# BioinfoMachineLearning/bio-diffusion

Hardware: NVIDIA H100
Metric: molecules/sec (1000-step sample) (higher is better)
Workload: dtype bf16x2 (split hi+lo operands, f32 accumulate; <=1e-4 of the fp32 reference)

## Files before the change

bio-diffusion_b200/csrc/bdiff_edge_tc.cuh:

```cuda
#pragma once
#include "bdiff_kernels.h"
#include "bdiff_slab.cuh"

namespace bdiff {

constexpr int TMT = 128;
constexpr int TC_SLOT = 2 * 160 * 32;
constexpr int TC_NSLOT = 5;
constexpr int TM_S = 0, TM_U0 = 256, TM_U1 = 288, TM_MV = 320, TM_VD0 = 416;
constexpr int TM_EX = 416, TM_EX_STRIDE = 40;

struct StreamSeg { int steps, rows, group; };
struct Stream { StreamSeg seg[8]; int n; };
__host__ __device__ constexpr int seg_step_bytes(StreamSeg g) { return 2 * g.rows * 32; }
__host__ __device__ constexpr int seg_chunks(StreamSeg g) { return (g.steps + g.group - 1) / g.group; }
__host__ __device__ constexpr size_t stream_bytes(const Stream& s) {
  size_t b = 0;
  for (int i = 0; i < s.n; ++i) b += (size_t)s.seg[i].steps * 2 * seg_step_bytes(s.seg[i]);
  return b;
}
__host__ __device__ constexpr long long stream_plane_rows(const Stream& s) {
  long long r = 0;
  for (int i = 0; i < s.n; ++i) r += (long long)s.seg[i].steps * 2 * s.seg[i].rows;
  return r;
}
__host__ __device__ constexpr int stream_max_chunk(const Stream& s) {
  int m = 0;
  for (int i = 0; i < s.n; ++i) {
    const int c = s.seg[i].group * seg_step_bytes(s.seg[i]);
    m = c > m ? c : m;
  }
  return m;
}

__host__ __device__ constexpr int tc_k0_steps(int Ed, int Xd) {
  return (Ed + (64 + Xd) / 4 + 9 + 15) / 16;
}
__host__ __device__ constexpr Stream tc_edge_stream(int k0s) {
  constexpr StreamSeg Ga{16, 160, 1}, Gb{2, 128, 1};
  return {{{k0s, 128, 1}, Ga, Gb, Ga, Gb, Ga, Gb, {16, 16, 4}}, 8};
}
static_assert(stream_max_chunk(tc_edge_stream(8)) <= TC_SLOT, "an edge-pass chunk must fit a ring slot");

struct TcBars {
  uint64_t full[TC_NSLOT], empty[TC_NSLOT], wbar;
  uint64_t item_full[2], item_empty[2], tile_done;
  alignas(16) int item[2][4];
};

constexpr int TC_EPI = 256;

struct alignas(16) SmallW {
  float Wd0x[16 * 20];
  float Wf0x[16 * 3];
  float Wu0[20 * 32];
  float Wdk[3][32 * 8];
  float Wfk[3][32 * 3];
  float Wuk[3][8 * 32];
  float bg[4][32];
  float bk[3][256];
  float wa[256];
  float ba[4];
};

struct EdgeTail : TcBars {
  float2 wbuf[2][8][2][32];
  SmallW sw;
  float sAttn[2][TMT];
  int sRow[TMT], sCol[TMT], sB[TMT], sNa[TMT];
  uint32_t winfo[8];
};

template <int HP, bool FIRST, bool LAST>
__device__ __forceinline__ void gate_update(int half, int ucol, const float* __restrict__ vdp,
                                            const float* __restrict__ Wu, const float* __restrict__ bgp,
                                            const float* __restrict__ Wdn, const float* __restrict__ Wfn,
                                            float* __restrict__ part) {
  float2 p2[4][3];
  if (!LAST) {
#pragma unroll
    for (int i = 0; i < 33; ++i) part[i] = 0.f;
#pragma unroll
    for (int hp = 0; hp < 4; ++hp) { p2[hp][0] = make_float2(0.f, 0.f); p2[hp][1] = p2[hp][0]; p2[hp][2] = p2[hp][0]; }
  }
  for (int oc = half * 2; oc < half * 2 + 2; ++oc) {
    float u[8], mv[24];
    scratch_ld<8>(ucol + oc * 8, u);
    if (!FIRST) scratch_ld<24>(TM_MV + oc * 24, mv);
#pragma unroll
    for (int jp = 0; jp < 4; ++jp) {
      const int o = oc * 8 + 2 * jp;
      const float2 g = sigmoid_acc2(__fadd2_rn(make_float2(u[2 * jp], u[2 * jp + 1]),
                                               *reinterpret_cast<const float2*>(bgp + o)));
      float2 s0 = make_float2(0.f, 0.f), s1 = s0, s2 = s0;
#pragma unroll
      for (int h = 0; h < HP; ++h) {
        const float2 wu = *reinterpret_cast<const float2*>(Wu + h * 32 + o);
        s0 = __ffma2_rn(wu, make_float2(vdp[h * 3 + 0], vdp[h * 3 + 0]), s0);
        s1 = __ffma2_rn(wu, make_float2(vdp[h * 3 + 1], vdp[h * 3 + 1]), s1);
        s2 = __ffma2_rn(wu, make_float2(vdp[h * 3 + 2], vdp[h * 3 + 2]), s2);
      }
      const int ja = 2 * jp * 3, jb = (2 * jp + 1) * 3;
      float2 r0, r1, r2;
      if (FIRST) { r0 = __fmul2_rn(s0, g); r1 = __fmul2_rn(s1, g); r2 = __fmul2_rn(s2, g); }
      else {
        r0 = __ffma2_rn(s0, g, make_float2(mv[ja + 0], mv[jb + 0]));
        r1 = __ffma2_rn(s1, g, make_float2(mv[ja + 1], mv[jb + 1]));
        r2 = __ffma2_rn(s2, g, make_float2(mv[ja + 2], mv[jb + 2]));
      }
      mv[ja + 0] = r0.x; mv[jb + 0] = r0.y; mv[ja + 1] = r1.x; mv[jb + 1] = r1.y; mv[ja + 2] = r2.x; mv[jb + 2] = r2.y;
    }
    scratch_st<24>(TM_MV + oc * 24, mv);
    if (!LAST) {
#pragma unroll
      for (int j = 0; j < 8; ++j) {
        const int c = oc * 8 + j;
        const float4 wd0 = *reinterpret_cast<const float4*>(Wdn + c * 8), wd1 = *reinterpret_cast<const float4*>(Wdn + c * 8 + 4);
        const float2 wdp[4] = {make_float2(wd0.x, wd0.y), make_float2(wd0.z, wd0.w), make_float2(wd1.x, wd1.y),
                               make_float2(wd1.z, wd1.w)};
#pragma unroll
        for (int x = 0; x < 3; ++x) {
          const float2 mb = make_float2(mv[j * 3 + x], mv[j * 3 + x]);
#pragma unroll
          for (int hp = 0; hp < 4; ++hp) p2[hp][x] = __ffma2_rn(wdp[hp], mb, p2[hp][x]);
        }
#pragma unroll
        for (int ch = 0; ch < 3; ++ch) {
          const float wf = Wfn[c * 3 + ch];
          part[24 + ch * 3 + 0] = fmaf(wf, mv[j * 3 + 0], part[24 + ch * 3 + 0]);
          part[24 + ch * 3 + 1] = fmaf(wf, mv[j * 3 + 1], part[24 + ch * 3 + 1]);
          part[24 + ch * 3 + 2] = fmaf(wf, mv[j * 3 + 2], part[24 + ch * 3 + 2]);
        }
      }
    }
  }
  if (!LAST) {
#pragma unroll
    for (int hp = 0; hp < 4; ++hp)
#pragma unroll
      for (int x = 0; x < 3; ++x) { part[(2 * hp) * 3 + x] = p2[hp][x].x; part[(2 * hp + 1) * 3 + x] = p2[hp][x].y; }
  }
}

__device__ __forceinline__ void pair_exchange33(int half, const float* __restrict__ mine, float* __restrict__ theirs) {
  float pad[40];
#pragma unroll
  for (int i = 0; i < 33; ++i) pad[i] = mine[i];
#pragma unroll
  for (int i = 33; i < 40; ++i) pad[i] = 0.f;
  scratch_st<40>(TM_EX + half * TM_EX_STRIDE, pad);
  named_bar_sync(3, TC_EPI);
  float got[40];
  scratch_ld<40>(TM_EX + (half ^ 1) * TM_EX_STRIDE, got);
#pragma unroll
  for (int i = 0; i < 33; ++i) theirs[i] = got[i];
}

}
```

bio-diffusion_b200/csrc/bdiff_layers_tc.cu:

```cuda
#include <type_traits>

#include "bdiff_node_tc.cuh"

namespace bdiff {

__device__ __forceinline__ int ld_acquire_gpu(const int* p) {
  int v;
  asm volatile("ld.acquire.gpu.global.s32 %0, [%1];" : "=r"(v) : "l"(p) : "memory");
  return v;
}
__device__ __forceinline__ void st_release_gpu(int* p, int v) {
  asm volatile("st.release.gpu.global.s32 [%0], %1;" ::"l"(p), "r"(v) : "memory");
}

union LayersTail {
  TcBars bars;
  EdgeTail edge;
  NodeTail node;
};
constexpr size_t LAYERS_SMEM_BYTES = XE_BLOCKS * (size_t)X_BLOCK + TC_NSLOT * (size_t)TC_SLOT + sizeof(LayersTail) + 1024;
static_assert(LAYERS_SMEM_BYTES + 64 <= 232448, "shared memory budget of the layer megakernel (227 KiB per block)");

constexpr int LAYERS_THREADS = 384;
constexpr int LAYERS_REG_COMPUTE = 232, LAYERS_REG_SERVICE = 40;
static_assert(256 * LAYERS_REG_COMPUTE + 128 * LAYERS_REG_SERVICE <= 168 * LAYERS_THREADS, "setmaxnreg pool");
constexpr int RING_CONSUMERS = TC_EPI / 32;

struct AccToScratch {};
template <int NS, int NU, class Issue, class Epi = AccToScratch>
__device__ __forceinline__ void run_seg(TcBars& B, uint32_t raddr, uint32_t& ci, int nch, int scol, bool sfresh, int ucol,
                                        int ufresh, Issue&& issue, Epi&& epi = Epi{}) {
  constexpr int RS = NS ? NS / 2 : 1, RU = NU ? NU / 2 : 1;
  const int wg = threadIdx.x >> 7;
  const bool lead = (threadIdx.x & 31) == 0;
  for (int h = 0; h < 2; ++h) {
    float s[RS], u[RU];
    if (NS) {
      if (sfresh) {
#pragma unroll
        for (int i = 0; i < RS; ++i) s[i] = 0.f;
      } else {
        acc_load<NS>(s, scol + h * NS, wg);
      }
    }
    if (NU) {
      if ((ufresh >> h) & 1) {
#pragma unroll
        for (int i = 0; i < RU; ++i) u[i] = 0.f;
      } else {
        acc_load<NU>(u, ucol + h * NU, wg);
      }
    }
    for (int c = 0; c < nch; ++c) {
      const uint32_t slot = ci % TC_NSLOT;
      float ts[RS], tu[RU];
#pragma unroll
      for (int i = 0; i < RS; ++i) ts[i] = 0.f;
#pragma unroll
      for (int i = 0; i < RU; ++i) tu[i] = 0.f;
      mbar_wait(&B.full[slot], (ci / TC_NSLOT) & 1);
      wgmma_fence();
      issue(ts, tu, raddr + slot * TC_SLOT, c);
      wgmma_commit();
      wgmma_wait<0>();
      acc_fence<RS>(ts);
      acc_fence<RU>(tu);
      mbar_arrive_if(&B.empty[slot], lead);
      ++ci;
      if (NS) {
#pragma unroll
        for (int i = 0; i < RS; ++i) s[i] += ts[i];
      }
      if (NU) {
#pragma unroll
        for (int i = 0; i < RU; ++i) u[i] += tu[i];
      }
    }
    if constexpr (std::is_same_v<std::decay_t<Epi>, AccToScratch>) {
      if (NS) acc_store<NS>(s, scol + h * NS, wg);
      if (NU) acc_store<NU>(u, ucol + h * NU, wg);
    } else {
      epi(s, u, h, wg);
    }
  }
}

template <int ED, int XD>
__global__ void __launch_bounds__(LAYERS_THREADS, 1) k_layers_tc(Plan p, Dims d, EmbedW ew, LayerSched q, Work w) {
  constexpr int HID0 = (64 + XD) / 4;
  constexpr int H2 = HID0 / 2;
  constexpr int K0RAW = ED + HID0 + 9;
  constexpr int K0S = (K0RAW + 15) / 16;
  static_assert(HID0 % 2 == 0 && H2 * 3 <= 32 && HID0 + 9 <= 32 && ED % 16 == 0, "layout");

  extern __shared__ unsigned char smem_raw[];
  unsigned char* smem = smem_raw + ((1024u - (smem_u32(smem_raw) & 1023u)) & 1023u);
  unsigned char* X = smem;
  unsigned char* ring = smem + XE_BLOCKS * X_BLOCK;
  unsigned char* tail = ring + TC_NSLOT * TC_SLOT;
  TcBars& B = *reinterpret_cast<TcBars*>(tail);
  const int tid = threadIdx.x, warp = __shfl_sync(0xffffffffu, tid >> 5, 0), lane = tid & 31;
  const int hid0 = d.hid0;
  const int per_layer = q.TE + q.TN;
  const int total_items = q.nitems;
  int* const flags = q.sched + 2;

  if (tid == 0) {
    for (int i = 0; i < TC_NSLOT; ++i) { mbar_init(&B.full[i], 1); mbar_init(&B.empty[i], RING_CONSUMERS); }
    for (int i = 0; i < 2; ++i) { mbar_init(&B.item_full[i], 1); mbar_init(&B.item_empty[i], TC_EPI + 1); }
    mbar_init(&B.tile_done, TC_EPI);
    mbar_init(&B.wbar, 1);
    mbar_fence_init();
    acc_scratch = w.acc + (size_t)blockIdx.x * TM_COLS * 128;
  }
  __syncthreads();

  if (warp == 8) {
    asm volatile("setmaxnreg.dec.sync.aligned.u32 %0;\n" ::"n"(LAYERS_REG_SERVICE));
    if (lane == 0) {
      uint32_t ci = 0;
      for (uint32_t k = 0;; ++k) {
        const uint32_t slot = k & 1;
        mbar_wait_backoff(&B.item_empty[slot], ((k >> 1) & 1) ^ 1);
        int type = -1, layer = 0, tile = 0;
        for (;;) {
          const int qi = atomicAdd(q.sched, 1);
          if (qi >= 2 * total_items) break;
          const int it = __ldg(q.items + (qi >> 1));
          type = (it >> 30) & 1; layer = (it >> 24) & 63; tile = 2 * (it & 0xffffff) + (qi & 1);
          if (tile < (type == 0 ? q.TE : q.TN)) break;
          type = -1;
        }
        B.item[slot][0] = type; B.item[slot][1] = layer; B.item[slot][2] = tile;
        mbar_arrive(&B.item_full[slot]);
        if (type < 0) break;
        const size_t stride = type == 0 ? q.edge_blob_stride : q.node_blob_stride;
        const unsigned char* blob = (type == 0 ? q.edge_blob : q.node_blob) + (size_t)layer * stride;
        const Stream S = type == 0 ? tc_edge_stream(K0S) : tc_node_stream(layer == q.L - 1);
        size_t off = 0;
        for (int i = 0; i < S.n; ++i) {
          const StreamSeg g = S.seg[i];
          const uint32_t step = seg_step_bytes(g);
          for (int h = 0; h < 2; ++h)
            for (int c = 0; c < seg_chunks(g); ++c) {
              const int steps = min(g.group, g.steps - c * g.group);
              const uint32_t s = ci % TC_NSLOT;
              mbar_wait_backoff(&B.empty[s], ((ci / TC_NSLOT) & 1) ^ 1);
              mbar_expect_tx(&B.full[s], steps * step);
              bulk_g2s(ring + s * TC_SLOT, blob + h * (stride / 2) + off + (size_t)c * g.group * step, steps * step, &B.full[s]);
              ++ci;
            }
          off += (size_t)g.steps * step;
        }
      }
    }
  } else if (warp == 9) {
    asm volatile("setmaxnreg.dec.sync.aligned.u32 %0;\n" ::"n"(LAYERS_REG_SERVICE));
    if (lane == 0) {
      for (uint32_t k = 0;; ++k) {
        const uint32_t slot = k & 1;
        mbar_wait(&B.item_full[slot], (k >> 1) & 1);
        const int type = B.item[slot][0], layer = B.item[slot][1], tile = B.item[slot][2];
        if (type < 0) break;
        mbar_wait_backoff(&B.tile_done, k & 1);
        __threadfence();
        st_release_gpu(flags + (size_t)layer * per_layer + (type == 0 ? tile : q.TE + tile), 1);
        mbar_arrive(&B.item_empty[slot]);
      }
    }
  } else if (warp >= 10) {
    asm volatile("setmaxnreg.dec.sync.aligned.u32 %0;\n" ::"n"(LAYERS_REG_SERVICE));
  } else {
    asm volatile("setmaxnreg.inc.sync.aligned.u32 %0;\n" ::"n"(LAYERS_REG_COMPUTE));
    uint32_t pw = 0, ci = 0;
    int cur_type = -1, cur_layer = -1;
    const uint32_t xa = smem_u32(X) + (uint32_t)(tid >> 7) * 8192u;
    const uint32_t raddr = smem_u32(ring);
    int es = 0;
    long long* stamp = nullptr;
    auto PH = [&]() __attribute__((always_inline)) { if (stamp && tid == 0 && es < 32) stamp[es] = clock64(); ++es; };
    bool stamped[2] = {false, false};
    auto sz = [](int n) { return (uint32_t)((n * 4 + 15) & ~15); };
    for (uint32_t k = 0;; ++k) {
      const uint32_t slot = k & 1;
      mbar_wait(&B.item_full[slot], (k >> 1) & 1);
      const int type = __shfl_sync(0xffffffffu, B.item[slot][0], 0);
      const int layer = __shfl_sync(0xffffffffu, B.item[slot][1], 0);
      const int tile = __shfl_sync(0xffffffffu, B.item[slot][2], 0);
      if (type < 0) break;
      if (tid == 0 && w.dbg && k < 16) {
        w.dbg[(size_t)blockIdx.x * 64 + 4 * k] = (type << 30) | (layer << 24) | tile;
        w.dbg[(size_t)blockIdx.x * 64 + 4 * k + 1] = clock64();
      }
      if (type != cur_type || layer != cur_layer) {
        named_bar_sync(3, TC_EPI);
        if (tid == 0) {
          const LayerW lw = q.layers[layer];
          auto stage = [&](auto&& list) {
            uint32_t total = 0;
            list([&](float*, const float*, int n) { total += sz(n); });
            mbar_expect_tx(&B.wbar, total);
            list([&](float* dst, const float* src, int n) { bulk_g2s(dst, src, sz(n), &B.wbar); });
          };
          if (type == 0) {
            SmallW& s = reinterpret_cast<EdgeTail*>(tail)->sw;
            stage([&](auto&& cp) {
              cp(s.Wd0x, lw.Wd0x, XD * HID0); cp(s.Wf0x, lw.Wf0x, XD * 3); cp(s.Wu0, lw.Wu0, HID0 * 32);
              for (int kk = 0; kk < 3; ++kk) {
                cp(s.Wdk[kk], lw.Wdk[kk], 256); cp(s.Wuk[kk], lw.Wuk[kk], 256); cp(s.bk[kk], lw.bk[kk], 256);
                cp(s.Wfk[kk], lw.Wfk[kk], 96); cp(s.bg[kk + 1], lw.bgk[kk], 32);
              }
              cp(s.bg[0], lw.bg0, 32); cp(s.wa, lw.wa, 256); cp(s.ba, lw.ba, 1);
            });
          } else {
            const int last = layer == q.L - 1;
            const LayerW wn = q.layers[last ? layer : layer + 1];
            SmallWR4& s = reinterpret_cast<NodeTail*>(tail)->sw;
            stage([&](auto&& cp) {
              cp(s.Wdf, lw.Wdf, 64 * 16); cp(s.Wff, lw.Wff, 64 * 3); cp(s.Wuf, lw.Wuf, 16 * 32); cp(s.bgf, lw.bgf, 32);
              cp(s.b1, lw.b1, 256); cp(s.b2, lw.b2, 256);
              cp(s.Wdp, lw.Wdp, 32 * 8); cp(s.Wfp, lw.Wfp, 32 * 3); cp(s.Wup, lw.Wup, 8); cp(s.bp, lw.bp, 256);
              cp(s.wgp, lw.Wgp, 256); cp(s.bgp, lw.bgp, 1);
              if (!last) {
                cp(s.u.nx.b0, wn.b0, 256);
                cp(s.u.nx.Wd0i, wn.Wd0i, 32 * hid0); cp(s.u.nx.Wd0j, wn.Wd0j, 32 * hid0);
                cp(s.u.nx.Wf0i, wn.Wf0i, 96); cp(s.u.nx.Wf0j, wn.Wf0j, 96);
              } else {
                cp(s.u.pj.pWd, ew.pWd, 32 * 32); cp(s.u.pj.pWf, ew.pWf, 96); cp(s.u.pj.pbs, ew.pbs, d.Hin);
              }
            });
          }
        }
        mbar_wait(&B.wbar, pw);
        pw ^= 1;
        cur_type = type; cur_layer = layer;
      }
      if (tid == 0) {
        int lo = 0, hi = -1;
        const int* fbase = flags;
        if (type == 0) {
          if (layer > 0) {
            const int2 dep = q.edge_dep[tile];
            lo = dep.x; hi = dep.y;
            fbase = flags + (size_t)(layer - 1) * per_layer + q.TE;
          }
        } else {
          const int2 dep = q.node_dep[tile];
          lo = dep.x; hi = dep.y;
          fbase = flags + (size_t)layer * per_layer;
        }
        const long long t0 = clock64();
        for (int u = lo; u <= hi; ++u) {
          while (ld_acquire_gpu(fbase + u) == 0) {
            if (clock64() - t0 > (1ll << 32)) { atomicExch(q.err, 1); __threadfence_system(); __trap(); }
          }
        }
      }
      named_bar_sync(3, TC_EPI);
      __threadfence();
      if (tid == 0 && w.dbg && k < 16) w.dbg[(size_t)blockIdx.x * 64 + 4 * k + 2] = clock64();
      es = 0;
      stamp = nullptr;
      if (w.dbg && k >= 2 && !stamped[type]) { stamp = w.dbg + 256 * 64 + (size_t)blockIdx.x * 64 + type * 32; stamped[type] = true; }
      PH();
      const int last = type == 1 && layer == q.L - 1;
      int ph = 0;
      auto gemm = [&](int phase) __attribute__((always_inline)) {
        if (type == 0) {
          const int ph = phase;
#include "edge_tile_mma.inc"
        } else {
          const int ph = phase;
#include "node_r4_tile_mma.inc"
        }
      };
      auto run = [&]() __attribute__((always_inline)) { fence_proxy_async(); named_bar_sync(3, TC_EPI); PH(); gemm(ph++); };
      auto publish = [&]() __attribute__((always_inline)) { run(); named_bar_sync(3, TC_EPI); PH(); };
      auto release_u = [&]() __attribute__((always_inline)) { named_bar_sync(3, TC_EPI); gemm(-1); named_bar_sync(3, TC_EPI); };
      if (type == 0) {
        EdgeTail& T = *reinterpret_cast<EdgeTail*>(tail);
        const int half = tid >> 7, r = tid & 127;
        const SmallW& sw = T.sw;
#include "edge_tile_epilogue.inc"
      } else {
        NodeTail& T = *reinterpret_cast<NodeTail*>(tail);
        NodeScratch& SC = *reinterpret_cast<NodeScratch*>(X + R5_BLOCKS * R5_BLOCK);
        const int l = lane, s = warp, c0 = warp * 32;
        const SmallWR4& sw = T.sw;
#include "node_r4_tile_epilogue.inc"
      }
      PH();
      if (tid == 0 && w.dbg && k < 16) w.dbg[(size_t)blockIdx.x * 64 + 4 * k + 3] = clock64();
      mbar_arrive(&B.tile_done);
      mbar_arrive(&B.item_empty[slot]);
    }
  }
  __syncthreads();
}

bool tc_supported(int Ed, int Xd) { return (Ed == 64 && Xd == 16) || (Ed == 16 && Xd == 8); }

cudaError_t tc_layers_configure() {
  cudaError_t e = cudaFuncSetAttribute(k_layers_tc<64, 16>, cudaFuncAttributeMaxDynamicSharedMemorySize,
                                       (int)LAYERS_SMEM_BYTES);
  if (e != cudaSuccess) return e;
  return cudaFuncSetAttribute(k_layers_tc<16, 8>, cudaFuncAttributeMaxDynamicSharedMemorySize, (int)LAYERS_SMEM_BYTES);
}

void launch_layers_tc(cudaStream_t st, const Plan& p, const Dims& d, const EmbedW& ew, const LayerSched& q,
                      const Work& w, int num_sms) {
  const int grid = 2 * q.nitems < num_sms ? 2 * q.nitems : num_sms;
  if (d.Ed == 64) k_layers_tc<64, 16><<<grid, LAYERS_THREADS, LAYERS_SMEM_BYTES, st>>>(p, d, ew, q, w);
  else k_layers_tc<16, 8><<<grid, LAYERS_THREADS, LAYERS_SMEM_BYTES, st>>>(p, d, ew, q, w);
}

}
```

bio-diffusion_b200/csrc/bdiff_tc_pack.cu:

```cuda
#include "bdiff_node_tc.cuh"

namespace bdiff {

size_t tc_blob_bytes(int Ed, int Xd) { return stream_bytes(tc_edge_stream(tc_k0_steps(Ed, Xd))); }
size_t tc_node_blob_bytes() { return stream_bytes(tc_node_stream(false)); }

struct SlabPos {
  int seg, rows;
  int k0, n;
  int half, local;
  size_t base;
};
__device__ bool stream_find(const Stream& S, long long row, SlabPos& p) {
  size_t base = 0;
  for (int i = 0; i < S.n; ++i) {
    const StreamSeg g = S.seg[i];
    const long long seg_rows = (long long)g.steps * 2 * g.rows;
    if (row >= seg_rows) {
      row -= seg_rows;
      base += (size_t)g.steps * seg_step_bytes(g);
      continue;
    }
    const int step = (int)(row / (2 * g.rows)), n = (int)(row % (2 * g.rows));
    const int body = g.rows < 128 ? g.rows : 128, gate = g.rows - body;
    p.seg = i; p.rows = g.rows; p.k0 = step * 16; p.n = n;
    p.base = base + (size_t)step * seg_step_bytes(g);
    if (n < 2 * body) { p.half = n / body; p.local = n % body; }
    else { p.half = (n - 2 * body) / gate; p.local = body + (n - 2 * body) % gate; }
    return true;
  }
  return false;
}

__global__ void k_pack_edge_slabs(LayerW lw, Dims d, unsigned char* __restrict__ blob, size_t half_bytes) {
  const Stream S = tc_edge_stream(tc_k0_steps(d.Ed, d.Xd));
  const long long idx = (long long)blockIdx.x * blockDim.x + threadIdx.x;
  const int kk = (int)(idx & 15);
  SlabPos p;
  if (!stream_find(S, idx >> 4, p)) return;
  const int n = p.n, k = p.k0 + kk;
  float v;
  if (p.seg == 0) {
    v = k < d.K0 ? lw.W0e[(size_t)k * 256 + n] : 0.f;
  } else if (p.seg == 7) {
    v = lw.Wgk[2][(size_t)k * 32 + n];
  } else {
    const int gi = (p.seg - 1) >> 1;
    if (!(p.seg & 1)) {
      v = 256 + k < kKM ? lw.Wk[gi][(size_t)(256 + k) * 256 + n] : 0.f;
    } else if (n < 256) {
      v = lw.Wk[gi][(size_t)k * 256 + n];
    } else {
      const float* wprev = gi == 0 ? lw.Wg0 : lw.Wgk[gi - 1];
      const float* wthis = lw.Wgk[gi];
      const bool odd = ((gi + 1) & 1) != 0;
      const int c = (n - 256) & 31;
      v = (p.half == 0) == odd ? wprev[(size_t)k * 32 + c] : -wthis[(size_t)k * 32 + c];
    }
  }
  slab_store(blob + (size_t)p.half * half_bytes + p.base, p.rows, p.local, kk, v);
}

__global__ void k_pack_node_slabs(LayerW lw, LayerW wn, EmbedW ew, Dims d, int last, unsigned char* __restrict__ blob,
                                  size_t half_bytes) {
  const Stream S = tc_node_stream(last);
  const long long idx = (long long)blockIdx.x * blockDim.x + threadIdx.x;
  const int kk = (int)(idx & 15);
  SlabPos p;
  if (!stream_find(S, idx >> 4, p)) return;
  const int n = p.n, k = p.k0 + kk;
  float v;
  switch (p.seg) {
    case NG_1A: v = lw.W1[(size_t)k * 256 + n]; break;
    case NG_1B: v = n < 256 ? lw.W1[(size_t)(256 + k) * 256 + n] : -lw.Wgf[(size_t)k * 32 + (n - 256)]; break;
    case NG_1C: v = 512 + k < kKFF ? lw.W1[(size_t)(512 + k) * 256 + n] : 0.f; break;
    case NG_2: v = lw.W2[(size_t)k * 256 + n]; break;
    case NG_3A: v = n < 256 ? lw.Wp[(size_t)k * 256 + n] : lw.Wgf[(size_t)k * 32 + (n - 256)]; break;
    default:
      if (p.seg == (last ? NGL_3B : NG_3B)) v = 256 + k < kKM ? lw.Wp[(size_t)(256 + k) * 256 + n] : 0.f;
      else if (last) v = (k < 300 && n < d.Hin) ? ew.pWs[(size_t)k * d.Hin + n] : 0.f;
      else v = (p.seg == NG_4 ? wn.Wsi : wn.Wsj)[(size_t)k * 256 + n];
  }
  slab_store(blob + (size_t)p.half * half_bytes + p.base, p.rows, p.local, kk, v);
}

void launch_tc_pack(cudaStream_t st, const LayerW& lw, const Dims& d, unsigned char* blob) {
  const long long total = stream_plane_rows(tc_edge_stream(tc_k0_steps(d.Ed, d.Xd))) * 16;
  k_pack_edge_slabs<<<(unsigned)((total + 255) / 256), 256, 0, st>>>(lw, d, blob, tc_blob_bytes(d.Ed, d.Xd) / 2);
}

void launch_tc_pack_node(cudaStream_t st, const LayerW& lw, const LayerW& wn, const EmbedW& ew, const Dims& d, int last,
                         unsigned char* blob) {
  const long long total = stream_plane_rows(tc_node_stream(last)) * 16;
  k_pack_node_slabs<<<(unsigned)((total + 255) / 256), 256, 0, st>>>(lw, wn, ew, d, last, blob, tc_node_blob_bytes() / 2);
}

}
```

bio-diffusion_b200/csrc/edge_tile_epilogue.inc:

```
      const long long g = (long long)tile * TMT + r;
      constexpr int PV = HID0 * 3 + 9, PF4 = (PV + 3) / 4, PLD = PF4 * 4 + 1;
      constexpr int XF4 = XD * 3 / 4, XLD = XD * 3 + 1;
      constexpr int C0 = 128;
      static_assert(K0S <= 8 && 64 * (PLD + XLD) * 4 <= 2 * X_BLOCK, "staging areas");
      auto sFp = [&](int rr) { return reinterpret_cast<float*>(X + (rr >> 6) * XE_LO * X_BLOCK) + (rr & 63) * PLD; };
      auto sFx = [&](int rr) { return reinterpret_cast<float*>(X + (rr >> 6) * XE_LO * X_BLOCK) + 64 * PLD + (rr & 63) * XLD; };
      const int4 rc = __ldg(p.edge_rc + g);
      float f[9];
      {
        constexpr int F4_ROW = ED / 4;
        const float4* eb = reinterpret_cast<const float4*>(w.e + (size_t)tile * TMT * ED);
        const float4* xb = reinterpret_cast<const float4*>(w.xi + (size_t)tile * TMT * XD * 3);
        float4 ev[TMT * F4_ROW / TC_EPI], xv[TMT * XF4 / TC_EPI];
#pragma unroll
        for (int i = 0; i < TMT * F4_ROW / TC_EPI; ++i) ev[i] = eb[i * TC_EPI + tid];
#pragma unroll
        for (int i = 0; i < TMT * XF4 / TC_EPI; ++i) xv[i] = xb[i * TC_EPI + tid];
#pragma unroll
        for (int qq = 0; qq < 9; ++qq) f[qq] = w.frames[(size_t)g * 9 + qq];
        if (half == 0) { T.sRow[r] = rc.x; T.sCol[r] = rc.y; T.sB[r] = rc.z; T.sNa[r] = rc.w; }
#pragma unroll
        for (int i = 0; i < TMT * F4_ROW / TC_EPI; ++i) {
          const int idx = i * TC_EPI + tid;
          const int rr = idx / F4_ROW, kk = (idx % F4_ROW) * 4;
          xe_store4(X, rr, C0 + kk, ev[i].x, ev[i].y, ev[i].z, ev[i].w);
        }
#pragma unroll
        for (int i = 0; i < TMT * XF4 / TC_EPI; ++i) {
          const int idx = i * TC_EPI + tid;
          float* dst = sFx(idx / XF4) + (idx % XF4) * 4;
          dst[0] = xv[i].x; dst[1] = xv[i].y; dst[2] = xv[i].z; dst[3] = xv[i].w;
        }
      }
      const int row = rc.x;
      const float* pi = w.PI + (size_t)(row < 0 ? 0 : row) * kPStride;
      named_bar_sync(3, TC_EPI);
      {
        float4 pv[(TMT * PF4 + TC_EPI - 1) / TC_EPI];
#pragma unroll
        for (int i = 0; i < (TMT * PF4 + TC_EPI - 1) / TC_EPI; ++i) {
          const int idx = i * TC_EPI + tid;
          pv[i] = make_float4(0.f, 0.f, 0.f, 0.f);
          if (idx < TMT * PF4) {
            const int rr = idx / PF4, cj = T.sCol[rr];
            if (cj >= 0) pv[i] = *reinterpret_cast<const float4*>(w.PJ + (size_t)cj * kPStride + kH + (idx - rr * PF4) * 4);
          }
        }
        float vdh[32], vdf0[9];
#pragma unroll
        for (int i = 0; i < 32; ++i) vdh[i] = 0.f;
#pragma unroll
        for (int i = 0; i < 9; ++i) vdf0[i] = 0.f;
        if (row >= 0) {
#pragma unroll
          for (int i = 0; i < H2 * 3; ++i) vdh[i] = pi[kH + half * H2 * 3 + i];
          if (half == 0) {
#pragma unroll
            for (int i = 0; i < 9; ++i) vdf0[i] = pi[kH + HID0 * 3 + i];
          }
        }
        float xi[XD * 3];
#pragma unroll
        for (int c = 0; c < XD * 3; ++c) xi[c] = sFx(r)[c];
#pragma unroll
        for (int i = 0; i < (TMT * PF4 + TC_EPI - 1) / TC_EPI; ++i) {
          const int idx = i * TC_EPI + tid;
          if (idx < TMT * PF4) {
            const int rr = idx / PF4;
            float* dst = sFp(rr) + (idx - rr * PF4) * 4;
            dst[0] = pv[i].x; dst[1] = pv[i].y; dst[2] = pv[i].z; dst[3] = pv[i].w;
          }
        }
        named_bar_sync(3, TC_EPI);
        const float* pjv = sFp(r);
#pragma unroll
        for (int i = 0; i < H2 * 3; ++i) vdh[i] += pjv[half * H2 * 3 + i];
        if (half == 0) {
#pragma unroll
          for (int i = 0; i < 9; ++i) vdf0[i] += pjv[HID0 * 3 + i];
        }
#pragma unroll
        for (int c = 0; c < XD; ++c) {
#pragma unroll
          for (int h = 0; h < H2; ++h) {
            const float wd = sw.Wd0x[c * HID0 + half * H2 + h];
            vdh[h * 3 + 0] = fmaf(wd, xi[c * 3 + 0], vdh[h * 3 + 0]);
            vdh[h * 3 + 1] = fmaf(wd, xi[c * 3 + 1], vdh[h * 3 + 1]);
            vdh[h * 3 + 2] = fmaf(wd, xi[c * 3 + 2], vdh[h * 3 + 2]);
          }
        }
#pragma unroll
        for (int h = 0; h < H2; ++h)
          xe_store1(X, r, C0 + ED + half * H2 + h, safe_norm3(vdh[h * 3], vdh[h * 3 + 1], vdh[h * 3 + 2]));
        scratch_st<32>(TM_VD0 + half * 32, vdh);
        if (half == 0) {
#pragma unroll
          for (int c = 0; c < XD; ++c)
#pragma unroll
            for (int ch = 0; ch < 3; ++ch) {
              const float wf = sw.Wf0x[c * 3 + ch];
              vdf0[ch * 3 + 0] = fmaf(wf, xi[c * 3 + 0], vdf0[ch * 3 + 0]);
              vdf0[ch * 3 + 1] = fmaf(wf, xi[c * 3 + 1], vdf0[ch * 3 + 1]);
              vdf0[ch * 3 + 2] = fmaf(wf, xi[c * 3 + 2], vdf0[ch * 3 + 2]);
            }
#pragma unroll
          for (int ch = 0; ch < 3; ++ch)
#pragma unroll
            for (int ax = 0; ax < 3; ++ax)
              xe_store1(X, r, C0 + ED + HID0 + ch * 3 + ax,
                        f[ax * 3] * vdf0[ch * 3] + f[ax * 3 + 1] * vdf0[ch * 3 + 1] + f[ax * 3 + 2] * vdf0[ch * 3 + 2]);
#pragma unroll
          for (int i = HID0 + 9; i < K0S * 16 - ED; ++i) xe_store1(X, r, C0 + ED + i, 0.f);
        }
      }
      run();
      publish();

      float vd[24], vdf[9];
      for (int k = 1; k <= 3; ++k) {
        float part[33], other[33];
        if (k == 1) {
          float vd0[HID0 * 3];
          {
            float t0[64];
            float* t1 = t0 + 32;
            scratch_ld<64>(TM_VD0, t0);
#pragma unroll
            for (int i = 0; i < H2 * 3; ++i) { vd0[i] = t0[i]; vd0[H2 * 3 + i] = t1[i]; }
          }
          named_bar_sync(3, TC_EPI);
          gate_update<HID0, true, false>(half, TM_U0, vd0, sw.Wu0, sw.bg[0], sw.Wdk[0], sw.Wfk[0], part);
        } else {
          gate_update<8, false, false>(half, ((k - 1) & 1) ? TM_U1 : TM_U0, vd, sw.Wuk[k - 2], sw.bg[k - 1],
                                       sw.Wdk[k - 1], sw.Wfk[k - 1], part);
        }
        pair_exchange33(half, part, other);
#pragma unroll
        for (int i = 0; i < 24; ++i) vd[i] = half == 0 ? part[i] + other[i] : other[i] + part[i];
#pragma unroll
        for (int i = 0; i < 9; ++i) vdf[i] = half == 0 ? part[24 + i] + other[24 + i] : other[24 + i] + part[24 + i];
        {
          float a[16];
          if (half == 0) {
#pragma unroll
            for (int h = 0; h < 8; ++h) a[h] = safe_norm3(vd[h * 3], vd[h * 3 + 1], vd[h * 3 + 2]);
#pragma unroll
            for (int i = 0; i < 8; ++i) {
              const int ch = i / 3, ax = i - ch * 3;
              a[8 + i] = f[ax * 3] * vdf[ch * 3] + f[ax * 3 + 1] * vdf[ch * 3 + 1] + f[ax * 3 + 2] * vdf[ch * 3 + 2];
            }
          } else {
            a[0] = f[6] * vdf[6] + f[7] * vdf[7] + f[8] * vdf[8];
#pragma unroll
            for (int i = 1; i < 16; ++i) a[i] = 0.f;
          }
          xe_store8_extra(X, r, half * 16, a);
          xe_store8_extra(X, r, half * 16 + 8, a + 8);
        }
        run();
        publish();
      }
      const int wr0 = warp * 16;
      uint32_t m_start, m_end;
      {
        const int li = lane & 15, tr = wr0 + li;
        const int rw = T.sRow[tr];
        const int rp = tr > 0 ? T.sRow[tr - 1] : -2;
        const int rn = tr < TMT - 1 ? T.sRow[tr + 1] : -2;
        m_start = __ballot_sync(0xffffffffu, rw != rp) & 0xffffu;
        m_end = __ballot_sync(0xffffffffu, rw != rn && rw >= 0) & 0xffffu;
        if (lane == 0) T.winfo[warp] = m_start | (m_end << 16);
      }
      named_bar_sync(3, TC_EPI);
      const bool cutL = T.sB[0] != 0;
      const bool cutR = T.sRow[TMT - 1] >= 0 && T.sB[TMT - 1] != T.sNa[TMT - 1] - 1;
      const bool cont_in = !(m_start & 1u);
      float attw[16];
#pragma unroll
      for (int i = 0; i < 16; ++i) attw[i] = sigmoid_acc(T.sAttn[0][wr0 + i] + T.sAttn[1][wr0 + i] + sw.ba[0]);
      auto emit = [&](int trow, float2 val, int t, bool active) {
        if (!active) return;
        const bool l = cutL && (T.sRow[trow] == T.sRow[0]);
        const bool rr_ = cutR && (T.sRow[trow] == T.sRow[TMT - 1]);
        const size_t col = (size_t)t * 64 + 2 * lane;
        if (l && rr_) *reinterpret_cast<float2*>(w.mid + (size_t)tile * kMsg + col) = val;
        else if (l || rr_) atomicAdd(reinterpret_cast<float2*>(w.agg + (size_t)T.sRow[trow] * kMsg + col), val);
        else *reinterpret_cast<float2*>(w.agg + (size_t)T.sRow[trow] * kMsg + col) = val;
      };
      auto finish_crossing = [&](int t, bool active) {
        if (!(cont_in && (m_end & 0xffffu))) return;
        const float2 (*wb)[2][32] = T.wbuf[t & 1];
        int wa = warp - 1;
        while (wa > 0 && !(T.winfo[wa] & 0xffffu) && !(T.winfo[wa] >> 16)) --wa;
        float2 s = wb[wa][1][lane];
        for (int v2 = wa + 1; v2 < warp; ++v2) s = __fadd2_rn(s, wb[v2][1][lane]);
        s = __fadd2_rn(s, wb[warp][0][lane]);
        emit(wr0 + (__ffs(m_end & 0xffffu) - 1), s, t, active);
      };
      for (int t = 0; t < 4; ++t) {
        const unsigned char* xh_ = X + t * X_BLOCK + (lane & 3) * 4;
        const unsigned char* xl_ = X + (XE_LO + t) * X_BLOCK + (lane & 3) * 4;
        float2 acc = make_float2(0.f, 0.f);
        bool from_prev = cont_in;
        uint32_t hw[16], lw_[16];
#pragma unroll
        for (int i = 0; i < 16; ++i) {
          const int row_ = wr0 + i;
          const uint32_t off = (uint32_t)row_ * 128u + ((((uint32_t)lane >> 2) ^ ((uint32_t)row_ & 7u)) << 4);
          hw[i] = *reinterpret_cast<const uint32_t*>(xh_ + off);
          lw_[i] = *reinterpret_cast<const uint32_t*>(xl_ + off);
        }
#pragma unroll
        for (int i = 0; i < 16; ++i) {
          const int row_ = wr0 + i;
          const float2 x = join_bf16x2(hw[i], lw_[i]);
          const float2 a2 = make_float2(attw[i], attw[i]);
          acc = ((m_start >> i) & 1u) ? __fmul2_rn(a2, x) : __ffma2_rn(a2, x, acc);
          if ((m_end >> i) & 1u) {
            if (from_prev) T.wbuf[t & 1][warp][0][lane] = acc;
            else emit(row_, acc, t, true);
            from_prev = false;
          }
        }
        if (!((m_end >> 15) & 1u)) T.wbuf[t & 1][warp][1][lane] = acc;
        named_bar_sync(3, TC_EPI);
        finish_crossing(t, true);
      }
      {
        float dummy[33];
        gate_update<8, false, true>(half, TM_U1, vd, sw.Wuk[2], sw.bg[3], nullptr, nullptr, dummy);
      }
      named_bar_sync(3, TC_EPI);
      float2* sRA = reinterpret_cast<float2*>(X + XE_EXTRA * X_BLOCK);
      float2* sRB = reinterpret_cast<float2*>(X);
      float2* sRw = wr0 < 64 ? sRA + wr0 * 32 : sRB + (wr0 - 64) * 32;
      float2* sRr = r < 64 ? sRA + r * 32 : sRB + (r - 64) * 32;
      for (int t = 4; t < 6; ++t) {
        {
          float v[32];
          if (t == 4) {
            scratch_ld<32>(TM_MV + half * 32, v);
#pragma unroll
            for (int k = 0; k < 16; ++k) sRr[half * 16 + (k ^ (r & 15))] = make_float2(v[2 * k], v[2 * k + 1]);
          } else {
            scratch_ld<16>(TM_MV + 64 + half * 16, v);
#pragma unroll
            for (int k = 0; k < 8; ++k) sRr[(half * 8 + k) ^ (r & 15)] = make_float2(v[2 * k], v[2 * k + 1]);
          }
        }
        named_bar_sync(3, TC_EPI);
        const bool active = t < 5 || lane < 16;
        {
          const int hb = (lane >> 4) * 16, kq = lane & 15;
          float2 acc = make_float2(0.f, 0.f);
          bool from_prev = cont_in;
          float2 xv[16];
#pragma unroll
          for (int i = 0; i < 16; ++i) xv[i] = sRw[i * 32 + hb + (kq ^ i)];
#pragma unroll
          for (int i = 0; i < 16; ++i) {
            const float2 x = xv[i];
            acc = ((m_start >> i) & 1u) ? x : __fadd2_rn(acc, x);
            if ((m_end >> i) & 1u) {
              if (from_prev) T.wbuf[t & 1][warp][0][lane] = acc;
              else emit(wr0 + i, acc, t, active);
              from_prev = false;
            }
          }
          if (!((m_end >> 15) & 1u)) T.wbuf[t & 1][warp][1][lane] = acc;
        }
        named_bar_sync(3, TC_EPI);
        finish_crossing(t, active);
      }
      named_bar_sync(3, TC_EPI);
```

bio-diffusion_b200/csrc/edge_tile_mma.inc:

```
        {
          auto adh = [&](int ks) { return gmma_desc_sw128(xa + (ks >> 2) * X_BLOCK + (ks & 3) * 32); };
          auto adl = [&](int ks) { return gmma_desc_sw128(xa + (XE_LO + (ks >> 2)) * X_BLOCK + (ks & 3) * 32); };
          auto bd = [](uint32_t b, int nl) { return gmma_desc_k16(b, nl * 16, 128); };
          EdgeTail& ET = *reinterpret_cast<EdgeTail*>(tail);
          constexpr Stream ES = tc_edge_stream(K0S);
          constexpr StreamSeg G0 = ES.seg[0], GA = ES.seg[1], GB = ES.seg[2], G4 = ES.seg[7];
          auto a_word = [&](int rr, int c) { return reinterpret_cast<uint32_t*>(X + (c >> 6) * X_BLOCK + sw128_offset(rr, c & 63)); };
          if (ph == 0) {
            run_seg<128, 0>(B, raddr, ci, seg_chunks(G0), TM_S, true, 0, 0, [&](float* s, float*, uint32_t wb, int ks) {
              const uint64_t h = bd(wb, 128), l = bd(wb + 128 * 32, 128);
              wgmma_n128<1>(s, adh(ks + 8), h); wgmma_n128<1>(s, adl(ks + 8), h); wgmma_n128<1>(s, adh(ks + 8), l);
            }, [&](float* s, float*, int h, int wg) __attribute__((always_inline)) {
              const float* pi[2];
              const float* pj[2];
#pragma unroll
              for (int r8 = 0; r8 < 2; ++r8) {
                const int rr = frag_row(wg, 2 * r8);
                const int ri = ET.sRow[rr], cj = ET.sCol[rr];
                const int rin = ri < 0 ? 0 : ri, cjn = cj < 0 ? 0 : cj;
                pi[r8] = w.PI + (size_t)rin * kPStride + h * 128;
                pj[r8] = w.PJT + ((size_t)(cjn >> 5) * 256 + h * 128) * 32 + (cjn & 31);
              }
#pragma unroll
              for (int j = 0; j < 64; j += 2) {
                const int r8 = (j >> 1) & 1, c = frag_col(j);
                const float2 pa = *reinterpret_cast<const float2*>(pi[r8] + c);
                const float v0 = s[j] + (pa.x + pj[r8][c * 32]), v1 = s[j + 1] + (pa.y + pj[r8][(c + 1) * 32]);
                const float2 m = silu_acc2(make_float2(v0, v1));
                const int rr = frag_row(wg, j), cc = h * 128 + c;
                uint32_t hi, lo;
                split_bf16x2(m.x, m.y, hi, lo);
                a_word(rr, cc)[0] = hi;
                a_word(rr, cc)[XE_LO * X_BLOCK / 4] = lo;
              }
            });
          } else if (ph == 7) {
            run_seg<0, 16>(B, raddr, ci, seg_chunks(G4), 0, false, TM_U1, 0, [&](float*, float* u, uint32_t wb, int c) {
#pragma unroll
              for (int s4 = 0; s4 < 4; ++s4) {
                const int ks = c * 4 + s4;
                const uint64_t h = bd(wb + s4 * 1024, 16), l = bd(wb + s4 * 1024 + 512, 16);
                wgmma_n16<1>(u, adh(ks), h); wgmma_n16<1>(u, adl(ks), h); wgmma_n16<1>(u, adh(ks), l);
              }
            });
          } else if (ph & 1) {
            const int k = (ph + 1) >> 1;
            run_seg<128, 32>(B, raddr, ci, seg_chunks(GA), TM_S, true, TM_U0, k == 1 ? 3 : 1 << (k & 1), [&](float* s, float* u, uint32_t wb, int ks) {
              const uint32_t bl = wb + GA.rows * 32;
              const uint64_t ah = adh(ks), al = adl(ks);
              wgmma_n128<1>(s, ah, bd(wb, GA.rows)); wgmma_n32<1>(u, ah, bd(wb + 128 * 16, GA.rows));
              wgmma_n128<1>(s, al, bd(wb, GA.rows)); wgmma_n32<1>(u, al, bd(wb + 128 * 16, GA.rows));
              wgmma_n128<1>(s, ah, bd(bl, GA.rows)); wgmma_n32<1>(u, ah, bd(bl + 128 * 16, GA.rows));
            });
          } else {
            const int k = ph >> 1;
            const uint32_t xe = xa + XE_EXTRA * X_BLOCK;
            run_seg<128, 0>(B, raddr, ci, seg_chunks(GB), TM_S, false, 0, 0, [&](float* s, float*, uint32_t wb, int ks) {
              const uint64_t ah = gmma_desc_sw128(xe + ks * 32), al = gmma_desc_sw128(xe + 64 + ks * 32);
              const uint64_t h = bd(wb, 128), l = bd(wb + 128 * 32, 128);
              wgmma_n128<1>(s, ah, h); wgmma_n128<1>(s, al, h); wgmma_n128<1>(s, ah, l);
            }, [&](float* s, float*, int h, int wg) __attribute__((always_inline)) {
              const float* bk = ET.sw.bk[k - 1] + h * 128;
#pragma unroll
              for (int j = 0; j < 64; j += 2) {
                const int rr = frag_row(wg, j), c = frag_col(j);
                uint32_t* wd = a_word(rr, h * 128 + c);
                const float2 m = join_bf16x2(wd[0], wd[XE_LO * X_BLOCK / 4]);
                const float2 mm = __fadd2_rn(m, silu_acc2(__fadd2_rn(make_float2(s[j], s[j + 1]),
                                                                     *reinterpret_cast<const float2*>(bk + c))));
                uint32_t hi, lo;
                split_bf16x2(mm.x, mm.y, hi, lo);
                wd[0] = hi;
                wd[XE_LO * X_BLOCK / 4] = lo;
                s[j] = mm.x; s[j + 1] = mm.y;
              }
              if (k == 3) {
                const float* wa = ET.sw.wa + h * 128;
                const int qb = threadIdx.x & 28;
                float2 a[2] = {make_float2(0.f, 0.f), make_float2(0.f, 0.f)};
#pragma unroll
                for (int g = 0; g < 16; ++g) {
                  const float2 wv = *reinterpret_cast<const float2*>(wa + frag_col(4 * g));
#pragma unroll
                  for (int q = 0; q < 4; ++q) {
#pragma unroll
                    for (int r8 = 0; r8 < 2; ++r8) {
                      const int j = 4 * g + 2 * r8;
                      const float2 t = __ffma2_rn(make_float2(s[j], s[j + 1]), wv, a[r8]);
                      a[r8] = make_float2(__shfl_sync(0xffffffffu, t.x, qb | q), __shfl_sync(0xffffffffu, t.y, qb | q));
                    }
                  }
                }
                ET.sAttn[h][frag_row(wg, 0)] = a[0].x + a[0].y;
                ET.sAttn[h][frag_row(wg, 2)] = a[1].x + a[1].y;
              }
            });
          }
        }
```

Baseline: 24.44.

## Restructure edge GEMM stream: separate gate-U segment and hold message accumulators in registers

The edge pass used to compute the 256-wide message GEMM in two parts. A fused 160-row segment produced S plus the gate U, S was spilled to TMEM/scratch, and it was later reloaded for a short 2-step extra-K segment. The stream is now split into a dedicated U segment that groups four k-steps per chunk, and an 18-step S segment that covers both the main and extra K ranges. That S segment uses a new run_seg_held, which keeps both 128-column halves of the accumulator in registers, so the S scratch round trip is gone. This raises register pressure (two 64-float accumulators held at once), reorders the weight packing, and moves the vd reduction into the loop after run().

Measured after the change: 25.80 (median of 6 runs). +5.6%, better.

```diff
diff --git a/bio-diffusion_b200/csrc/bdiff_edge_tc.cuh b/bio-diffusion_b200/csrc/bdiff_edge_tc.cuh
--- a/bio-diffusion_b200/csrc/bdiff_edge_tc.cuh
+++ b/bio-diffusion_b200/csrc/bdiff_edge_tc.cuh
@@ -7,7 +7,7 @@
 constexpr int TMT = 128;
 constexpr int TC_SLOT = 2 * 160 * 32;
 constexpr int TC_NSLOT = 5;
-constexpr int TM_S = 0, TM_U0 = 256, TM_U1 = 288, TM_MV = 320, TM_VD0 = 416;
+constexpr int TM_U0 = 256, TM_U1 = 288, TM_MV = 320, TM_VD0 = 416;
 constexpr int TM_EX = 416, TM_EX_STRIDE = 40;
 
 struct StreamSeg { int steps, rows, group; };
@@ -37,8 +37,8 @@
   return (Ed + (64 + Xd) / 4 + 9 + 15) / 16;
 }
 __host__ __device__ constexpr Stream tc_edge_stream(int k0s) {
-  constexpr StreamSeg Ga{16, 160, 1}, Gb{2, 128, 1};
-  return {{{k0s, 128, 1}, Ga, Gb, Ga, Gb, Ga, Gb, {16, 16, 4}}, 8};
+  constexpr StreamSeg Gu{16, 32, 4}, Gs{18, 128, 1};
+  return {{{k0s, 128, 1}, Gu, Gs, Gu, Gs, Gu, Gs, {16, 16, 4}}, 8};
 }
 static_assert(stream_max_chunk(tc_edge_stream(8)) <= TC_SLOT, "an edge-pass chunk must fit a ring slot");
 
diff --git a/bio-diffusion_b200/csrc/bdiff_layers_tc.cu b/bio-diffusion_b200/csrc/bdiff_layers_tc.cu
--- a/bio-diffusion_b200/csrc/bdiff_layers_tc.cu
+++ b/bio-diffusion_b200/csrc/bdiff_layers_tc.cu
@@ -26,13 +26,42 @@
 static_assert(256 * LAYERS_REG_COMPUTE + 128 * LAYERS_REG_SERVICE <= 168 * LAYERS_THREADS, "setmaxnreg pool");
 constexpr int RING_CONSUMERS = TC_EPI / 32;
 
+template <int NS, int NU, int TU, class Issue>
+__device__ __forceinline__ void seg_chunk(TcBars& B, uint32_t raddr, uint32_t& ci, int c, float* s, float* u, Issue& issue) {
+  constexpr int RS = NS ? NS / 2 : 1, RU = NU ? NU / 2 : 1;
+  const uint32_t slot = ci % TC_NSLOT;
+  float ts[RS], tu[TU * RU];
+#pragma unroll
+  for (int i = 0; i < RS; ++i) ts[i] = 0.f;
+#pragma unroll
+  for (int i = 0; i < TU * RU; ++i) tu[i] = 0.f;
+  mbar_wait(&B.full[slot], (ci / TC_NSLOT) & 1);
+  wgmma_fence();
+  issue(ts, tu, raddr + slot * TC_SLOT, c);
+  wgmma_commit();
+  wgmma_wait<0>();
+  acc_fence<RS>(ts);
+  acc_fence<TU * RU>(tu);
+  mbar_arrive_if(&B.empty[slot], (threadIdx.x & 31) == 0);
+  ++ci;
+  if (NS) {
+#pragma unroll
+    for (int i = 0; i < RS; ++i) s[i] += ts[i];
+  }
+  if (NU) {
+#pragma unroll
+    for (int t = 0; t < TU; ++t)
+#pragma unroll
+      for (int i = 0; i < RU; ++i) u[i] += tu[t * RU + i];
+  }
+}
+
 struct AccToScratch {};
-template <int NS, int NU, class Issue, class Epi = AccToScratch>
+template <int NS, int NU, int TU = 1, class Issue, class Epi = AccToScratch>
 __device__ __forceinline__ void run_seg(TcBars& B, uint32_t raddr, uint32_t& ci, int nch, int scol, bool sfresh, int ucol,
                                         int ufresh, Issue&& issue, Epi&& epi = Epi{}) {
   constexpr int RS = NS ? NS / 2 : 1, RU = NU ? NU / 2 : 1;
   const int wg = threadIdx.x >> 7;
-  const bool lead = (threadIdx.x & 31) == 0;
   for (int h = 0; h < 2; ++h) {
     float s[RS], u[RU];
     if (NS) {
@@ -51,31 +80,7 @@
         acc_load<NU>(u, ucol + h * NU, wg);
       }
     }
-    for (int c = 0; c < nch; ++c) {
-      const uint32_t slot = ci % TC_NSLOT;
-      float ts[RS], tu[RU];
-#pragma unroll
-      for (int i = 0; i < RS; ++i) ts[i] = 0.f;
-#pragma unroll
-      for (int i = 0; i < RU; ++i) tu[i] = 0.f;
-      mbar_wait(&B.full[slot], (ci / TC_NSLOT) & 1);
-      wgmma_fence();
-      issue(ts, tu, raddr + slot * TC_SLOT, c);
-      wgmma_commit();
-      wgmma_wait<0>();
-      acc_fence<RS>(ts);
-      acc_fence<RU>(tu);
-      mbar_arrive_if(&B.empty[slot], lead);
-      ++ci;
-      if (NS) {
-#pragma unroll
-        for (int i = 0; i < RS; ++i) s[i] += ts[i];
-      }
-      if (NU) {
-#pragma unroll
-        for (int i = 0; i < RU; ++i) u[i] += tu[i];
-      }
-    }
+    for (int c = 0; c < nch; ++c) seg_chunk<NS, NU, TU>(B, raddr, ci, c, s, u, issue);
     if constexpr (std::is_same_v<std::decay_t<Epi>, AccToScratch>) {
       if (NS) acc_store<NS>(s, scol + h * NS, wg);
       if (NU) acc_store<NU>(u, ucol + h * NU, wg);
@@ -83,6 +88,22 @@
       epi(s, u, h, wg);
     }
   }
+}
+
+template <class Issue, class Epi>
+__device__ __forceinline__ void run_seg_held(TcBars& B, uint32_t raddr, uint32_t& ci, int nch, int hold, Issue&& issue,
+                                             Epi&& epi) {
+  const int wg = threadIdx.x >> 7;
+  float s0[64], s1[64];
+#pragma unroll
+  for (int i = 0; i < 64; ++i) s0[i] = 0.f;
+  for (int c = 0; c < nch; ++c) seg_chunk<128, 0, 1>(B, raddr, ci, c, s0, nullptr, issue);
+#pragma unroll
+  for (int i = 0; i < 64; ++i) s1[i] = 0.f;
+  for (int c = 0; c <= hold; ++c) seg_chunk<128, 0, 1>(B, raddr, ci, c, s1, nullptr, issue);
+  epi(s0, nullptr, 0, wg);
+  for (int c = hold + 1; c < nch; ++c) seg_chunk<128, 0, 1>(B, raddr, ci, c, s1, nullptr, issue);
+  epi(s1, nullptr, 1, wg);
 }
 
 template <int ED, int XD>
diff --git a/bio-diffusion_b200/csrc/bdiff_tc_pack.cu b/bio-diffusion_b200/csrc/bdiff_tc_pack.cu
--- a/bio-diffusion_b200/csrc/bdiff_tc_pack.cu
+++ b/bio-diffusion_b200/csrc/bdiff_tc_pack.cu
@@ -47,14 +47,12 @@
   } else {
     const int gi = (p.seg - 1) >> 1;
     if (!(p.seg & 1)) {
-      v = 256 + k < kKM ? lw.Wk[gi][(size_t)(256 + k) * 256 + n] : 0.f;
-    } else if (n < 256) {
-      v = lw.Wk[gi][(size_t)k * 256 + n];
+      v = k < kKM ? lw.Wk[gi][(size_t)k * 256 + n] : 0.f;
     } else {
       const float* wprev = gi == 0 ? lw.Wg0 : lw.Wgk[gi - 1];
       const float* wthis = lw.Wgk[gi];
       const bool odd = ((gi + 1) & 1) != 0;
-      const int c = (n - 256) & 31;
+      const int c = n & 31;
       v = (p.half == 0) == odd ? wprev[(size_t)k * 32 + c] : -wthis[(size_t)k * 32 + c];
     }
   }
diff --git a/bio-diffusion_b200/csrc/edge_tile_epilogue.inc b/bio-diffusion_b200/csrc/edge_tile_epilogue.inc
--- a/bio-diffusion_b200/csrc/edge_tile_epilogue.inc
+++ b/bio-diffusion_b200/csrc/edge_tile_epilogue.inc
@@ -116,9 +116,11 @@
       run();
       publish();
 
-      float vd[24], vdf[9];
+      float vd[24];
       for (int k = 1; k <= 3; ++k) {
-        float part[33], other[33];
+        float part[33], other[33], vdf[9];
+#pragma unroll
+        for (int qq = 0; qq < 9; ++qq) f[qq] = w.frames[(size_t)g * 9 + qq];
         if (k == 1) {
           float vd0[HID0 * 3];
           {
@@ -158,6 +160,13 @@
           xe_store8_extra(X, r, half * 16 + 8, a + 8);
         }
         run();
+        {
+          float t0[24], t1[24];
+          scratch_ld<24>(TM_EX, t0);
+          scratch_ld<24>(TM_EX + TM_EX_STRIDE, t1);
+#pragma unroll
+          for (int i = 0; i < 24; ++i) vd[i] = t0[i] + t1[i];
+        }
         publish();
       }
       const int wr0 = warp * 16;
diff --git a/bio-diffusion_b200/csrc/edge_tile_mma.inc b/bio-diffusion_b200/csrc/edge_tile_mma.inc
--- a/bio-diffusion_b200/csrc/edge_tile_mma.inc
+++ b/bio-diffusion_b200/csrc/edge_tile_mma.inc
@@ -4,10 +4,12 @@
           auto bd = [](uint32_t b, int nl) { return gmma_desc_k16(b, nl * 16, 128); };
           EdgeTail& ET = *reinterpret_cast<EdgeTail*>(tail);
           constexpr Stream ES = tc_edge_stream(K0S);
-          constexpr StreamSeg G0 = ES.seg[0], GA = ES.seg[1], GB = ES.seg[2], G4 = ES.seg[7];
+          constexpr StreamSeg G0 = ES.seg[0], GU = ES.seg[1], GS = ES.seg[2], G4 = ES.seg[7];
+          static_assert(GU.rows == 32 && GU.group == 4 && GU.steps % 4 == 0 && GS.rows == 128 && GS.steps == 18 && GS.group == 1,
+                        "edge stream: the GEMM bodies below take these shapes");
           auto a_word = [&](int rr, int c) { return reinterpret_cast<uint32_t*>(X + (c >> 6) * X_BLOCK + sw128_offset(rr, c & 63)); };
           if (ph == 0) {
-            run_seg<128, 0>(B, raddr, ci, seg_chunks(G0), TM_S, true, 0, 0, [&](float* s, float*, uint32_t wb, int ks) {
+            run_seg<128, 0>(B, raddr, ci, seg_chunks(G0), 0, true, 0, 0, [&](float* s, float*, uint32_t wb, int ks) {
               const uint64_t h = bd(wb, 128), l = bd(wb + 128 * 32, 128);
               wgmma_n128<1>(s, adh(ks + 8), h); wgmma_n128<1>(s, adl(ks + 8), h); wgmma_n128<1>(s, adh(ks + 8), l);
             }, [&](float* s, float*, int h, int wg) __attribute__((always_inline)) {
@@ -45,18 +47,21 @@
             });
           } else if (ph & 1) {
             const int k = (ph + 1) >> 1;
-            run_seg<128, 32>(B, raddr, ci, seg_chunks(GA), TM_S, true, TM_U0, k == 1 ? 3 : 1 << (k & 1), [&](float* s, float* u, uint32_t wb, int ks) {
-              const uint32_t bl = wb + GA.rows * 32;
-              const uint64_t ah = adh(ks), al = adl(ks);
-              wgmma_n128<1>(s, ah, bd(wb, GA.rows)); wgmma_n32<1>(u, ah, bd(wb + 128 * 16, GA.rows));
-              wgmma_n128<1>(s, al, bd(wb, GA.rows)); wgmma_n32<1>(u, al, bd(wb + 128 * 16, GA.rows));
-              wgmma_n128<1>(s, ah, bd(bl, GA.rows)); wgmma_n32<1>(u, ah, bd(bl + 128 * 16, GA.rows));
+            run_seg<0, 32, 4>(B, raddr, ci, seg_chunks(GU), 0, false, TM_U0, k == 1 ? 3 : 1 << (k & 1), [&](float*, float* u, uint32_t wb, int c) {
+#pragma unroll
+              for (int s4 = 0; s4 < 4; ++s4) {
+                const int ks = c * 4 + s4;
+                const uint64_t ah = adh(ks), h = bd(wb + s4 * 2048, 32), l = bd(wb + s4 * 2048 + 1024, 32);
+                wgmma_n32<1>(u + s4 * 16, ah, h); wgmma_n32<1>(u + s4 * 16, adl(ks), h); wgmma_n32<1>(u + s4 * 16, ah, l);
+              }
             });
           } else {
             const int k = ph >> 1;
             const uint32_t xe = xa + XE_EXTRA * X_BLOCK;
-            run_seg<128, 0>(B, raddr, ci, seg_chunks(GB), TM_S, false, 0, 0, [&](float* s, float*, uint32_t wb, int ks) {
-              const uint64_t ah = gmma_desc_sw128(xe + ks * 32), al = gmma_desc_sw128(xe + 64 + ks * 32);
+            run_seg_held(B, raddr, ci, seg_chunks(GS), (128 / 16 - 1) / GS.group, [&](float* s, float*, uint32_t wb, int ks) {
+              const bool ext = ks >= 16;
+              const uint64_t ah = ext ? gmma_desc_sw128(xe + (ks - 16) * 32) : adh(ks);
+              const uint64_t al = ext ? gmma_desc_sw128(xe + 64 + (ks - 16) * 32) : adl(ks);
               const uint64_t h = bd(wb, 128), l = bd(wb + 128 * 32, 128);
               wgmma_n128<1>(s, ah, h); wgmma_n128<1>(s, al, h); wgmma_n128<1>(s, ah, l);
             }, [&](float* s, float*, int h, int wg) __attribute__((always_inline)) {
```
